# volume-em/empanada

Measured on AMD Instinct MI355X. Metric: Mvox/s end-to-end 3D panoptic inference (incl. consensus); PQ vs CPU ref, higher is better.
Workload: dtype f32

## Files before the change

empanada_amd/csrc/emp_conv.hip:

```cpp
#include "emp_common.h"
#include "emp_wino4.h"
#include <stdlib.h>

typedef float f32x16 __attribute__((ext_vector_type(16)));

#define CG_BM 128
#define CG_BK 32
#define CG_THREADS 256

struct ConvGeom {
    const float *x, *w, *scale, *shift, *res;
    float *out;
    int N, H, W, Cin, OH, OW, Cout, KH, KW, stride, pad, dil, relu;
    int64_t M, out_ps, res_ps;
    int tiles_m, tiles_n;
    int64_t x_bs, w_bs, out_bs;
    const int32_t *tiles;
    const float *proj_w;
    float *proj_out;
    int proj_n;
    int64_t hw;
};

__device__ __attribute__((aligned(16))) float cg_zero_page[64];
// ... 416 lines not shown
            }
            if constexpr (PROJ) {
                float ps[4] = {0.f, 0.f, 0.f, 0.f};
                if (valid && co + 3 < g.Cout) {
#pragma unroll
                    for (int q = 0; q < 4; ++q)
                        if (q < g.proj_n) {
                            const float4 wq = *reinterpret_cast<const float4 *>(g.proj_w + (int64_t)q * g.Cout + co);
                            ps[q] = __fadd_rn(__fadd_rn(__fadd_rn(__fmul_rn(v[0], wq.x), __fmul_rn(v[1], wq.y)),
                                                        __fmul_rn(v[2], wq.z)), __fmul_rn(v[3], wq.w));
                        }
                }
                *reinterpret_cast<float4 *>(&Cs[lrow_c * CLD + ccol]) = make_float4(ps[0], ps[1], ps[2], ps[3]);
            }
        }
        if constexpr (PROJ) {
            __syncthreads();
            for (int idx = tid; idx < EPI_ROWS * g.proj_n; idx += CG_THREADS) {
                const int row_l = idx / g.proj_n, q = idx - row_l * g.proj_n;
                const int64_t p = m0 + rd * EPI_ROWS + row_l;
                if (p < g.M) {
                    float t = Cs[row_l * CLD + q];
#pragma unroll 8
                    for (int j = 1; j < C4; ++j) t = __fadd_rn(t, Cs[row_l * CLD + 4 * j + q]);
                    const int64_t img = p / g.hw;
                    atomicAdd(g.proj_out + (img * g.proj_n + q) * g.hw + (p - img * g.hw), t);
                }
            }
        }
    }
}

struct CgPlan {
    bool narrow, respf, glds;
    int slab, tiles_m, tiles_n;
};

static CgPlan cg_plan(int64_t M, int Cout, int batch, bool has_res, bool res_vec_ok, bool may_split_n = true, int cin = 32)
{
    CgPlan p;
    const int64_t wide_blocks = emp_cdiv(M, CG_BM) * emp_cdiv(Cout, 128) * batch;
    p.narrow = Cout <= 64 || (Cout % 128 != 0 && Cout % 128 <= 64 && Cout < 512) || (may_split_n && wide_blocks < 256);
    p.tiles_m = (int)emp_cdiv(M, CG_BM);
    p.tiles_n = (int)emp_cdiv(Cout, p.narrow ? 64 : 128);
    static const char *fnarrow = getenv("EMP_CONV_NARROW");
    static const char *norespf = getenv("EMP_CONV_NO_RESPF");
    if (fnarrow && fnarrow[0] == '1') {
        p.narrow = true;
        p.tiles_n = (int)emp_cdiv(Cout, 64);
    }
    p.respf = has_res && res_vec_ok && Cout % (p.narrow ? 64 : 128) == 0 && !norespf;
    static const char *force = getenv("EMP_CONV_BK");
    const int64_t blocks = (int64_t)p.tiles_m * p.tiles_n * batch;
    p.slab = blocks > 512 ? 16 : 32;
    if (force && force[0] == '1') p.slab = 16;
    if (force && force[0] == '3') p.slab = 32;
    if (p.respf) p.slab = 32;
    if (cin % 32 != 0) {
        p.slab = 16;
        p.respf = false;
    }
    static const char *noglds = getenv("EMP_CONV_NO_GLDS");
    p.glds = !noglds;
    return p;
}

extern "C" int emp_conv_k_slab(int64_t M, int Cout, int batch, int has_residual)
{
    return cg_plan(M, Cout, batch, has_residual != 0, true).slab;
}

extern "C" int emp_conv_k_slab_cin(int64_t M, int Cout, int batch, int has_residual, int Cin)
{
    return cg_plan(M, Cout, batch, has_residual != 0, true, true, Cin).slab;
}

extern "C" __attribute__((visibility("hidden"))) int emp_conv1x1_ws_kind(int64_t M, int Cin, int Cout, int KH, int KW, int stride, int pad, int relu, int has_residual);
extern "C" __attribute__((visibility("hidden"))) int emp_conv1x1_ws_launch(int kind, const float *x, const float *w, const float *scale, const float *shift,
                                     const float *res, int64_t res_ps, int relu, int64_t M, int Cin, int Cout,
                                     float *out, int64_t out_ps, void *stream);
extern "C" __attribute__((visibility("hidden"))) int emp_gemm_ws_eligible(int batch, int64_t M, int N, int K, int slab);
extern "C" __attribute__((visibility("hidden"))) int emp_gemm_ws_launch(const float *A, const float *B, int batch, int64_t M, int N, int K, float *C,
                                                                        void *stream);

extern "C" int emp_conv_k_slab_geom(int64_t M, int Cout, int has_residual, int Cin, int KH, int KW, int stride, int pad,
                                    int relu)
{
    if (emp_conv1x1_ws_kind(M, Cin, Cout, KH, KW, stride, pad, relu, has_residual) == 1) return 64;
    return cg_plan(M, Cout, 1, has_residual != 0 && relu != 2, true, true, Cin).slab;
}

extern "C" int emp_conv_bn_act_nhwc(const float *x, const float *w_okkc, const float *scale, const float *shift,
                                    const float *residual, int64_t res_pixel_stride, int relu, int N, int H, int W,
                                    int Cin, int Cout, int KH, int KW, int stride, int pad, int dil, float *out,
                                    int64_t out_pixel_stride, void *stream)
{
    EMP_REQUIRE(x && w_okkc && out, "conv: null pointer");
    EMP_REQUIRE(N >= 0 && H > 0 && W > 0 && Cin > 0 && Cout > 0, "conv: bad shape");
    EMP_REQUIRE(Cin % 16 == 0, "conv: Cin %d must be a multiple of 16", Cin);
    EMP_REQUIRE(relu != 2 || residual, "conv: the gate epilogue (relu == 2) needs the gated tensor as residual");
    EMP_REQUIRE(KH >= 1 && KW >= 1 && KH <= 7 && KW <= 7 && stride >= 1 && dil >= 1 && pad >= 0, "conv: bad filter geometry");
    const int OH = (H + 2 * pad - dil * (KH - 1) - 1) / stride + 1;
    const int OW = (W + 2 * pad - dil * (KW - 1) - 1) / stride + 1;
    EMP_REQUIRE(OH > 0 && OW > 0, "conv: empty output");
    if (out_pixel_stride == 0) out_pixel_stride = Cout;
    if (res_pixel_stride == 0) res_pixel_stride = Cout;
    EMP_REQUIRE(out_pixel_stride >= Cout && res_pixel_stride >= Cout, "conv: bad pixel stride");
    EMP_REQUIRE(((reinterpret_cast<uintptr_t>(x) | reinterpret_cast<uintptr_t>(w_okkc)) & 15) == 0,
                "conv: x and w must be 16-byte aligned");
    EMP_REQUIRE(out != x, "conv: output cannot alias the input");
    if (N == 0) return EMP_OK;
    ConvGeom g;
    g.x = x; g.w = w_okkc; g.scale = scale; g.shift = shift; g.res = residual; g.out = out;
    g.N = N; g.H = H; g.W = W; g.Cin = Cin; g.OH = OH; g.OW = OW; g.Cout = Cout; g.KH = KH; g.KW = KW;
    g.stride = stride; g.pad = pad; g.dil = dil; g.relu = relu;
    g.M = (int64_t)N * OH * OW; g.out_ps = out_pixel_stride; g.res_ps = res_pixel_stride;
    g.x_bs = g.w_bs = g.out_bs = 0; g.tiles = nullptr; g.proj_w = nullptr; g.proj_out = nullptr; g.proj_n = 0; g.hw = 1;
    const bool res_vec_ok = (res_pixel_stride & 3) == 0 && (reinterpret_cast<uintptr_t>(residual) & 15) == 0;
    const bool io_vec_ok = res_vec_ok && (out_pixel_stride & 3) == 0 && (reinterpret_cast<uintptr_t>(out) & 15) == 0 &&
                           (!scale || (reinterpret_cast<uintptr_t>(scale) & 15) == 0) &&
                           (!shift || (reinterpret_cast<uintptr_t>(shift) & 15) == 0);
    const int ws = io_vec_ok && scale && shift ? emp_conv1x1_ws_kind(g.M, Cin, Cout, KH, KW, stride, pad, relu, residual != nullptr) : 0;
    if (ws == 1)
        return emp_conv1x1_ws_launch(1, x, w_okkc, scale, shift, residual, res_pixel_stride, relu, g.M, Cin, Cout, out,
                                     out_pixel_stride, stream);
    const CgPlan pl = cg_plan(g.M, Cout, 1, residual != nullptr && relu != 2, res_vec_ok, true, Cin);
    if (ws == 2 && !residual && pl.slab == 16)
        return emp_conv1x1_ws_launch(2, x, w_okkc, scale, shift, nullptr, res_pixel_stride, relu, g.M, Cin, Cout, out,
                                     out_pixel_stride, stream);
    if (ws == 3 && residual && pl.respf && pl.slab == 32 &&
        res_pixel_stride < (1 << 24) && out_pixel_stride < (1 << 24))
        return emp_conv1x1_ws_launch(3, x, w_okkc, scale, shift, residual, res_pixel_stride, relu, g.M, Cin, Cout, out,
                                     out_pixel_stride, stream);
    const bool narrow = pl.narrow, respf = pl.respf, bk16 = pl.slab == 16;
    EMP_REQUIRE((int64_t)pl.tiles_m * pl.tiles_n < (1LL << 28), "conv: too many tiles");
    g.tiles_m = pl.tiles_m;
    g.tiles_n = pl.tiles_n;
    const int T = g.tiles_m * g.tiles_n;
    const int grid = 8 * ((T + 7) / 8);
#define CG_GO(NT_, RES_, BK_, GL_) hipLaunchKernelGGL((conv_igemm_f32_kernel<NT_, 0, RES_, BK_, false, GL_>), dim3(grid), dim3(CG_THREADS), 0, emp_stream(stream), g)
#define CG_GATE(NT_, BK_) hipLaunchKernelGGL((conv_igemm_f32_kernel<NT_, 0, false, BK_, false, true, true>), dim3(grid), dim3(CG_THREADS), 0, emp_stream(stream), g)
    if (relu == 2) {
        if (narrow) { if (bk16) CG_GATE(1, 16); else CG_GATE(1, 32); }
        else { if (bk16) CG_GATE(2, 16); else CG_GATE(2, 32); }
    } else if (narrow) {
        if (respf) { if (pl.glds) CG_GO(1, true, 32, true); else CG_GO(1, true, 32, false); }
        else if (pl.glds) { if (bk16) CG_GO(1, false, 16, true); else CG_GO(1, false, 32, true); }
        else { if (bk16) CG_GO(1, false, 16, false); else CG_GO(1, false, 32, false); }
    } else {
        if (respf) { if (pl.glds) CG_GO(2, true, 32, true); else CG_GO(2, true, 32, false); }
        else if (pl.glds) { if (bk16) CG_GO(2, false, 16, true); else CG_GO(2, false, 32, true); }
        else { if (bk16) CG_GO(2, false, 16, false); else CG_GO(2, false, 32, false); }
    }
#undef CG_GO
#undef CG_GATE
    EMP_CHECK_LAUNCH("emp_conv_bn_act_nhwc");
    return EMP_OK;
}

__global__ __launch_bounds__(256) void splitk_reduce_kernel(const float *__restrict__ work, int nz, int64_t M, int Cout,
                                                            const float *__restrict__ scale,
                                                            const float *__restrict__ shift,
                                                            const float *__restrict__ res, int64_t res_ps, int relu,
                                                            float *__restrict__ out, int64_t out_ps)
{
    const int C4 = Cout >> 2;
// ... 33 lines not shown
    const int S = KH * KW * (Cin / 32);
    if (tiles > 128) return 1;
    int64_t k = 256 / tiles;
    if (k > S / 4) k = S / 4;
    if (k > 32) k = 32;
    return k >= 2 ? (int)k : 1;
}

extern "C" int emp_conv_splitk_bn_act_nhwc(const float *x, const float *w_okkc, const float *scale, const float *shift,
                                           const float *residual, int64_t res_pixel_stride, int relu, int N, int H, int W,
                                           int Cin, int Cout, int KH, int KW, int stride, int pad, int dil, int k_splits,
                                           float *work, float *out, int64_t out_pixel_stride, void *stream)
{
    EMP_REQUIRE(x && w_okkc && out && work, "conv_splitk: null pointer");
    EMP_REQUIRE(N >= 0 && H > 0 && W > 0 && Cin > 0 && Cout > 0, "conv_splitk: bad shape");
    EMP_REQUIRE(Cin % 32 == 0 && Cout % 4 == 0, "conv_splitk: Cin %d must be a multiple of 32, Cout %d of 4", Cin, Cout);
    EMP_REQUIRE(relu == 0 || relu == 1, "conv_splitk: relu must be 0 or 1");
    EMP_REQUIRE(KH >= 1 && KW >= 1 && KH <= 7 && KW <= 7 && stride >= 1 && dil >= 1 && pad >= 0, "conv_splitk: bad filter geometry");
    const int OH = (H + 2 * pad - dil * (KH - 1) - 1) / stride + 1;
    const int OW = (W + 2 * pad - dil * (KW - 1) - 1) / stride + 1;
    EMP_REQUIRE(OH > 0 && OW > 0, "conv_splitk: empty output");
    const int S = KH * KW * (Cin / 32);
    EMP_REQUIRE(k_splits >= 1 && k_splits <= S && k_splits <= 64, "conv_splitk: k_splits %d not in 1..min(%d, 64)", k_splits, S);
    if (out_pixel_stride == 0) out_pixel_stride = Cout;
    if (res_pixel_stride == 0) res_pixel_stride = Cout;
    EMP_REQUIRE(out_pixel_stride >= Cout && res_pixel_stride >= Cout, "conv_splitk: bad pixel stride");
    EMP_REQUIRE(((reinterpret_cast<uintptr_t>(x) | reinterpret_cast<uintptr_t>(w_okkc) | reinterpret_cast<uintptr_t>(work) |
                  reinterpret_cast<uintptr_t>(out) | reinterpret_cast<uintptr_t>(residual) | reinterpret_cast<uintptr_t>(scale) |
                  reinterpret_cast<uintptr_t>(shift)) & 15) == 0 && (out_pixel_stride & 3) == 0 && (res_pixel_stride & 3) == 0,
                "conv_splitk: pointers must be 16-byte aligned, pixel strides multiples of 4");
    EMP_REQUIRE(out != x && work != x && work != out, "conv_splitk: buffers must not alias");
    if (N == 0) return EMP_OK;
    ConvGeom g;
    g.x = x; g.w = w_okkc; g.scale = nullptr; g.shift = nullptr; g.res = nullptr; g.out = work;
    g.N = N; g.H = H; g.W = W; g.Cin = Cin; g.OH = OH; g.OW = OW; g.Cout = Cout; g.KH = KH; g.KW = KW;
    g.stride = stride; g.pad = pad; g.dil = dil; g.relu = 0;
    g.M = (int64_t)N * OH * OW; g.out_ps = Cout; g.res_ps = Cout;
    g.x_bs = g.w_bs = g.out_bs = 0; g.tiles = nullptr; g.proj_w = nullptr; g.proj_out = nullptr; g.proj_n = 0; g.hw = 1;
    const CgPlan pl = cg_plan(g.M, Cout, 1, false, true, true, Cin);
    EMP_REQUIRE((int64_t)pl.tiles_m * pl.tiles_n < (1LL << 28), "conv_splitk: too many tiles");
    g.tiles_m = pl.tiles_m;
    g.tiles_n = pl.tiles_n;
    const int T = g.tiles_m * g.tiles_n;
    const dim3 grid(8 * ((T + 7) / 8), 1, k_splits);
    hipStream_t st = emp_stream(stream);
    if (pl.narrow)
        hipLaunchKernelGGL((conv_igemm_f32_kernel<1, 0, false, 32, false, true>), grid, dim3(CG_THREADS), 0, st, g);
    else
        hipLaunchKernelGGL((conv_igemm_f32_kernel<2, 0, false, 32, false, true>), grid, dim3(CG_THREADS), 0, st, g);
    EMP_CHECK_LAUNCH("emp_conv_splitk_bn_act_nhwc(partials)");
    const int64_t total = g.M * (Cout / 4);
    hipLaunchKernelGGL(splitk_reduce_kernel, dim3(emp_grid(total, 256, 4096)), dim3(256), 0, st, work, k_splits, g.M, Cout,
                       scale, shift, residual, res_pixel_stride, relu, out, out_pixel_stride);
    EMP_CHECK_LAUNCH("emp_conv_splitk_bn_act_nhwc(reduce)");
    return EMP_OK;
}

extern "C" int emp_conv_bn_act_proj_nhwc(const float *x, const float *w_okkc, const float *scale, const float *shift,
                                         int relu, int N, int H, int W, int Cin, int Cout, int KH, int KW, int stride,
                                         int pad, int dil, const float *proj_w, int proj_n, float *proj_out,
                                         float *out, int64_t out_pixel_stride, void *stream)
{
    EMP_REQUIRE(x && w_okkc && proj_w && proj_out, "conv_proj: null pointer");
    EMP_REQUIRE(N >= 0 && H > 0 && W > 0 && Cin > 0 && Cin % CG_BK == 0, "conv_proj: bad shape (Cin %% %d)", CG_BK);
    EMP_REQUIRE(Cout == 128 || Cout == 256, "conv_proj: Cout %d must be 128 or 256 (at most two cout tiles)", Cout);
    EMP_REQUIRE(proj_n >= 1 && proj_n <= 4, "conv_proj: proj_n %d not in 1..4", proj_n);
    EMP_REQUIRE(KH >= 1 && KW >= 1 && KH <= 7 && KW <= 7 && stride >= 1 && dil >= 1 && pad >= 0, "conv_proj: bad filter geometry");
    const int OH = (H + 2 * pad - dil * (KH - 1) - 1) / stride + 1;
    const int OW = (W + 2 * pad - dil * (KW - 1) - 1) / stride + 1;
    EMP_REQUIRE(OH > 0 && OW > 0, "conv_proj: empty output");
    if (out_pixel_stride == 0) out_pixel_stride = Cout;
    EMP_REQUIRE(((reinterpret_cast<uintptr_t>(x) | reinterpret_cast<uintptr_t>(w_okkc) | reinterpret_cast<uintptr_t>(proj_w) |
                  reinterpret_cast<uintptr_t>(out)) & 15) == 0 && (out_pixel_stride & 3) == 0, "conv_proj: alignment");
    EMP_REQUIRE(out != x, "conv_proj: output cannot alias the input");
    if (N == 0) return EMP_OK;
    ConvGeom g;
    g.x = x; g.w = w_okkc; g.scale = scale; g.shift = shift; g.res = nullptr; g.out = out;
    g.N = N; g.H = H; g.W = W; g.Cin = Cin; g.OH = OH; g.OW = OW; g.Cout = Cout; g.KH = KH; g.KW = KW;
    g.stride = stride; g.pad = pad; g.dil = dil; g.relu = relu;
    g.M = (int64_t)N * OH * OW; g.out_ps = out_pixel_stride; g.res_ps = Cout;
    g.x_bs = g.w_bs = g.out_bs = 0; g.tiles = nullptr;
    g.proj_w = proj_w; g.proj_out = proj_out; g.proj_n = proj_n; g.hw = (int64_t)OH * OW;
    const CgPlan pl = cg_plan(g.M, Cout, 1, false, true, false);
    g.tiles_m = pl.tiles_m;
    g.tiles_n = pl.tiles_n;
    const int T = g.tiles_m * g.tiles_n;
    const int grid = 8 * ((T + 7) / 8);
#define CG_GOP(BK_, GL_) hipLaunchKernelGGL((conv_igemm_f32_kernel<2, 0, false, BK_, true, GL_>), dim3(grid), dim3(CG_THREADS), 0, emp_stream(stream), g)
    if (pl.glds) { if (pl.slab == 16) CG_GOP(16, true); else CG_GOP(32, true); }
    else { if (pl.slab == 16) CG_GOP(16, false); else CG_GOP(32, false); }
#undef CG_GOP
    EMP_CHECK_LAUNCH("emp_conv_bn_act_proj_nhwc");
    return EMP_OK;
}


__global__ __launch_bounds__(256) void wino_input_kernel(const float *__restrict__ x, const int32_t *__restrict__ tiles,
                                                         int64_t T, int H, int W, int C4, int dil, float4 *__restrict__ V)
{
    const int64_t total = T * C4;
    for (int64_t i = (int64_t)blockIdx.x * blockDim.x + threadIdx.x; i < total; i += (int64_t)gridDim.x * blockDim.x) {
        const int c4 = (int)(i % C4);
        const int64_t t = i / C4;
        const int n = tiles[3 * t], by = tiles[3 * t + 1], bx = tiles[3 * t + 2];
        const float4 *src = reinterpret_cast<const float4 *>(x) + (int64_t)n * H * W * C4 + c4;
        float4 d[4][4];
#pragma unroll
        for (int a = 0; a < 4; ++a)
#pragma unroll
            for (int b = 0; b < 4; ++b) {
                const int yy = by + a * dil, xx = bx + b * dil;
                d[a][b] = make_float4(0.f, 0.f, 0.f, 0.f);
                if (yy >= 0 && yy < H && xx >= 0 && xx < W) d[a][b] = src[((int64_t)yy * W + xx) * C4];
            }
#define W_SUB(p, q) make_float4(__fsub_rn(p.x, q.x), __fsub_rn(p.y, q.y), __fsub_rn(p.z, q.z), __fsub_rn(p.w, q.w))
#define W_ADD(p, q) make_float4(__fadd_rn(p.x, q.x), __fadd_rn(p.y, q.y), __fadd_rn(p.z, q.z), __fadd_rn(p.w, q.w))
        float4 tt[4][4];
#pragma unroll
        for (int a = 0; a < 4; ++a) {
            tt[a][0] = W_SUB(d[a][0], d[a][2]);
            tt[a][1] = W_ADD(d[a][1], d[a][2]);
            tt[a][2] = W_SUB(d[a][2], d[a][1]);
            tt[a][3] = W_SUB(d[a][1], d[a][3]);
        }
        float4 *dst = V + t * C4 + c4;
        const int64_t ps = T * C4;
#pragma unroll
        for (int v = 0; v < 4; ++v) {
            dst[(0 * 4 + v) * ps] = W_SUB(tt[0][v], tt[2][v]);
            dst[(1 * 4 + v) * ps] = W_ADD(tt[1][v], tt[2][v]);
            dst[(2 * 4 + v) * ps] = W_SUB(tt[2][v], tt[1][v]);
            dst[(3 * 4 + v) * ps] = W_SUB(tt[1][v], tt[3][v]);
        }
    }
}

__global__ __launch_bounds__(256) void wino_output_kernel(const float4 *__restrict__ Mw, const int32_t *__restrict__ tiles,
                                                          int64_t T, int H, int W, int Co4, int dil,
                                                          const float4 *__restrict__ scale, const float4 *__restrict__ shift,
                                                          int relu, float *__restrict__ out, int64_t out_ps)
{
    const int64_t total = T * Co4;
    for (int64_t i = (int64_t)blockIdx.x * blockDim.x + threadIdx.x; i < total; i += (int64_t)gridDim.x * blockDim.x) {
        const int c4 = (int)(i % Co4);
        const int64_t t = i / Co4;
        const int n = tiles[3 * t], oy = tiles[3 * t + 1] + dil, ox = tiles[3 * t + 2] + dil;
        const float4 *src = Mw + t * Co4 + c4;
        const int64_t ps = T * Co4;
        float4 m[4][4];
#pragma unroll
        for (int a = 0; a < 4; ++a)
#pragma unroll
            for (int b = 0; b < 4; ++b) m[a][b] = src[(a * 4 + b) * ps];
        float4 s[2][4];
#pragma unroll
        for (int b = 0; b < 4; ++b) {
            s[0][b] = W_ADD(W_ADD(m[0][b], m[1][b]), m[2][b]);
            s[1][b] = W_SUB(W_SUB(m[1][b], m[2][b]), m[3][b]);
        }
        float4 sc = make_float4(1.f, 1.f, 1.f, 1.f), sh = make_float4(0.f, 0.f, 0.f, 0.f);
        if (scale) sc = scale[c4];
        if (shift) sh = shift[c4];
#pragma unroll
        for (int a = 0; a < 2; ++a) {
            float4 yv[2];
            yv[0] = W_ADD(W_ADD(s[a][0], s[a][1]), s[a][2]);
// ... 367 lines not shown
```

empanada_amd/csrc/emp_conv1x1.hip:

```cpp
#include "emp_common.h"
#include <stdlib.h>
#include <atomic>
#include <type_traits>

typedef float f32x16 __attribute__((ext_vector_type(16)));
template <int V> using IC = std::integral_constant<int, V>;

#define PW_THREADS 256
#define PW_ROWS 32
#define PW_MIN_ROWS 65536
#define PW_MIN_ROWS_PLAN 262144

struct PwGeom {
    const float *x, *w, *scale, *shift, *res;
    float *out;
    int64_t M, out_ps, res_ps;
    int Cin, Cout, relu, groups, pix_blocks;
    int batch;
    int64_t x_bs, w_bs, out_bs;
};

template <int KS, int S, int CT, int PT, bool GEMM, bool RES, bool RELU, int MODE = 0>
__global__ __launch_bounds__(PW_THREADS, 1) void conv1x1_ws_kernel(PwGeom g)
{
    static_assert(MODE == 0 || RES, "MODE 1 is a residual form");
    constexpr int CIN = 64 * KS;
    constexpr int LD = CIN + 4;
    constexpr int BN = 32 * CT;
    constexpr int NQ = CIN / 8;
    constexpr int QS = S / 8;
    constexpr int ROWS = PW_ROWS * PT;
    static_assert(!RES || (CT == 4 && PT == 1 && !GEMM), "residual: 128-cout groups of the convolution form only");
    static_assert(S == 16 || S == 32 || S == 64, "K-slab");
    __shared__ __attribute__((aligned(16))) float Bs[BN * LD];

    const int bid = blockIdx.x;
    const int xcd = bid & 7, slot = bid >> 3;
    const int per_xcd = g.pix_blocks >> 3;
    const int gi = slot % g.groups;
    const int pb = xcd * per_xcd + slot / g.groups;
    const int n0 = GEMM ? 0 : gi * BN;
    const int tid = threadIdx.x;
    const float *xb = g.x, *wb = g.w;
    float *ob = g.out;

    auto stage = [&]() {
        for (int idx = tid; idx < BN * (CIN / 4); idx += PW_THREADS) {
            const int rr = idx / (CIN / 4), k4 = idx - rr * (CIN / 4);
            const int cw = n0 + CT * (rr & 31) + (rr >> 5);
            *reinterpret_cast<float4 *>(&Bs[rr * LD + 4 * k4]) = *reinterpret_cast<const float4 *>(wb + (int64_t)cw * CIN + 4 * k4);
        }
        __syncthreads();
    };

    const int wave = MODE != 0 ? __builtin_amdgcn_readfirstlane(tid >> 6) : tid >> 6, lane = tid & 63;
    const int r = lane & 31, hh = lane >> 5;
    const int co = n0 + CT * r;
    float sc[CT], sh[CT];
    if constexpr (!GEMM) {
        if constexpr (CT == 4) {
            { const float4 t = *reinterpret_cast<const float4 *>(g.scale + co); sc[0] = t.x; sc[1] = t.y; sc[2] = t.z; sc[3] = t.w; }
            { const float4 t = *reinterpret_cast<const float4 *>(g.shift + co); sh[0] = t.x; sh[1] = t.y; sh[2] = t.z; sh[3] = t.w; }
        } else {
            { const float2 t = *reinterpret_cast<const float2 *>(g.scale + co); sc[0] = t.x; sc[1] = t.y; }
            { const float2 t = *reinterpret_cast<const float2 *>(g.shift + co); sh[0] = t.x; sh[1] = t.y; }
        }
    }

    const int64_t n_tiles = (g.M + ROWS - 1) / ROWS;
    const int64_t n_full = g.M / ROWS;
    const float *Bl = &Bs[r * LD + hh * (S / 2)];
    const int64_t ops = GEMM ? (int64_t)BN : g.out_ps;
    const unsigned a_lane = r * CIN + hh * (S / 2);
    const unsigned r_lane = (unsigned)(4 * hh * g.res_ps + co), o_lane = (unsigned)(4 * hh * ops + co);

    auto load_a = [&](int64_t t, float4 (&a)[PT][NQ], const float *base) {
#pragma unroll
        for (int p = 0; p < PT; ++p) {
            const int64_t pa = t * ROWS + PW_ROWS * p + r;
            const float *ap = base + pa * CIN + hh * (S / 2);
#pragma unroll
            for (int i = 0; i < NQ; ++i) a[p][i] = *reinterpret_cast<const float4 *>(ap + S * (i / QS) + 4 * (i % QS));
        }
    };
    auto load_rs = [&](int64_t t, float4 (&rs)[RES ? 16 : 1]) {
        if constexpr (MODE == 1) {
            const float *rp = g.res + t * ROWS * g.res_ps;
#pragma unroll
            for (int q = 0; q < 16; ++q)
                rs[q] = *reinterpret_cast<const float4 *>(rp + (int64_t)((q & 3) + 8 * (q >> 2)) * g.res_ps + r_lane);
        } else if constexpr (RES) {
            const float *rp = g.res + (t * ROWS + 4 * hh) * g.res_ps + co;
#pragma unroll
            for (int q = 0; q < 16; ++q)
                rs[q] = *reinterpret_cast<const float4 *>(rp + (int64_t)((q & 3) + 8 * (q >> 2)) * g.res_ps);
        }
    };
    auto mma = [&](f32x16 (&acc)[PT * CT], const auto &a, auto i_lo_c, auto i_hi_c, auto a_off_c) {
        constexpr int i_lo = decltype(i_lo_c)::value, i_hi = decltype(i_hi_c)::value;
        constexpr int a_off = decltype(a_off_c)::value;
        if constexpr (i_lo == 0) {
#pragma unroll
            for (int j = 0; j < PT * CT; ++j)
#pragma unroll
                for (int q = 0; q < 16; ++q) acc[j][q] = 0.f;
        }
        int opaque = 0;
        asm volatile("" : "+v"(opaque));
        const float *Bt = Bl + opaque;
#pragma unroll
        for (int i = i_lo; i < i_hi; ++i) {
            float4 b[CT];
#pragma unroll
            for (int j = 0; j < CT; ++j) b[j] = *reinterpret_cast<const float4 *>(Bt + j * 32 * LD + S * (i / QS) + 4 * (i % QS));
#pragma unroll
            for (int e = 0; e < 4; ++e)
#pragma unroll
                for (int p = 0; p < PT; ++p) {
                    const float av = e == 0 ? a[p][i - a_off].x : e == 1 ? a[p][i - a_off].y : e == 2 ? a[p][i - a_off].z : a[p][i - a_off].w;
#pragma unroll
                    for (int j = 0; j < CT; ++j) {
                        const float bv = e == 0 ? b[j].x : e == 1 ? b[j].y : e == 2 ? b[j].z : b[j].w;
                        acc[p * CT + j] = __builtin_amdgcn_mfma_f32_32x32x2f32(av, bv, acc[p * CT + j], 0, 0, 0);
                    }
                }
        }
    };
    auto mma_all = [&](f32x16 (&acc)[PT * CT], const float4 (&a)[PT][NQ]) { mma(acc, a, IC<0>{}, IC<NQ>{}, IC<0>{}); };
    auto put = [&](float *dst, const f32x16 (&acc)[PT * CT], int p, const float4 (&rs)[RES ? 16 : 1], int q) {
        float v[CT];
#pragma unroll
        for (int e = 0; e < CT; ++e) v[e] = acc[p * CT + e][q];
        if constexpr (!GEMM) {
#pragma unroll
            for (int e = 0; e < CT; ++e) v[e] = __fadd_rn(__fmul_rn(v[e], sc[e]), sh[e]);
        }
        if constexpr (RES) {
            v[0] = __fadd_rn(v[0], rs[q].x); v[1] = __fadd_rn(v[1], rs[q].y);
            v[2] = __fadd_rn(v[2], rs[q].z); v[3] = __fadd_rn(v[3], rs[q].w);
        }
        if constexpr (RELU) {
#pragma unroll
            for (int e = 0; e < CT; ++e) v[e] = fmaxf(v[e], 0.f);
        }
        if constexpr (CT == 4) *reinterpret_cast<float4 *>(dst) = make_float4(v[0], v[1], v[2], v[3]);
        else *reinterpret_cast<float2 *>(dst) = make_float2(v[0], v[1]);
    };
    auto epi_part = [&](const f32x16 (&acc)[PT * CT], const float4 (&rs)[RES ? 16 : 1], int64_t t, auto q0_c, auto q1_c) {
#pragma unroll
        for (int p = 0; p < PT; ++p) {
            float *op = MODE != 0 ? ob + (t * ROWS + PW_ROWS * p) * ops : ob + (t * ROWS + PW_ROWS * p + 4 * hh) * ops + co;
#pragma unroll
            for (int q = decltype(q0_c)::value; q < decltype(q1_c)::value; ++q)
                put(op + (int64_t)((q & 3) + 8 * (q >> 2)) * ops + (MODE != 0 ? o_lane : 0u), acc, p, rs, q);
        }
    };
    auto epi = [&](const f32x16 (&acc)[PT * CT], const float4 (&rs)[RES ? 16 : 1], int64_t t) { epi_part(acc, rs, t, IC<0>{}, IC<16>{}); };

    auto run = [&](const int64_t t_first, const int64_t stride_t, const int64_t t_end) {
        const int64_t f_end = n_full < t_end ? n_full : t_end;
        if (t_first < f_end) {
            const int64_t m = (f_end - t_first + stride_t - 1) / stride_t;
            auto tile = [&](int64_t i) { return t_first + (i < m ? i : m - 1) * stride_t; };
            if constexpr (MODE == 0) {
                float4 a0[PT][NQ], a1[PT][NQ], rs0[RES ? 16 : 1], rs1[RES ? 16 : 1];
                f32x16 acc0[PT * CT], acc1[PT * CT];
                load_a(tile(0), a0, xb);
                load_rs(tile(0), rs0);
                load_a(tile(1), a1, xb);
                mma_all(acc0, a0);
                int64_t i = 1;
                for (; i + 1 < m; i += 2) {
                    load_rs(tile(i), rs1);
                    load_a(tile(i + 1), a0, xb);
                    mma_all(acc1, a1);
                    epi(acc0, rs0, tile(i - 1));
                    load_rs(tile(i + 1), rs0);
                    load_a(tile(i + 2), a1, xb);
                    mma_all(acc0, a0);
                    epi(acc1, rs1, tile(i));
                }
                if (i < m) {
                    load_rs(tile(i), rs1);
                    mma_all(acc1, a1);
                    epi(acc0, rs0, tile(i - 1));
                    epi(acc1, rs1, tile(i));
                } else {
                    epi(acc0, rs0, tile(i - 1));
                }
            } else if constexpr (MODE == 1) {
                constexpr int NE = NQ / 8;
                float4 a[PT][4 * NE], rs[16];
                f32x16 acc0[PT * CT], acc1[PT * CT];
                auto load_k = [&](int64_t t, auto slab_c) {
                    constexpr int off = decltype(slab_c)::value * NE, slot = (decltype(slab_c)::value & 3) * NE;
#pragma unroll
                    for (int p = 0; p < PT; ++p) {
                        const float *ap = xb + (t * ROWS + PW_ROWS * p) * CIN + a_lane;
#pragma unroll
                        for (int k = 0; k < NE; ++k) a[p][slot + k] = *reinterpret_cast<const float4 *>(ap + S * ((off + k) / QS) + 4 * ((off + k) % QS));
                    }
                };
                auto phase = [&](f32x16 (&acc_n)[PT * CT], int64_t t_n, const f32x16 (&acc_o)[PT * CT], int64_t t_o, auto with_epi, int64_t t_x, auto with_next) {
                    if constexpr (decltype(with_epi)::value) load_rs(t_o, rs);
                    auto eighth = [&](auto e_c) {
                        constexpr int E = decltype(e_c)::value;
                        mma(acc_n, a, IC<NE * E>{}, IC<NE * E + NE>{}, IC<NE * (E & 4)>{});
                        if constexpr (decltype(with_epi)::value && E >= 4) epi_part(acc_o, rs, t_o, IC<4 * (E - 4)>{}, IC<4 * (E - 4) + 4>{});
                        __builtin_amdgcn_sched_barrier(0);
                        if constexpr (E < 4) load_k(t_n, IC<E + 4>{});
                        else if constexpr (decltype(with_next)::value) load_k(t_x, IC<E - 4>{});
                    };
                    eighth(IC<0>{}); eighth(IC<1>{}); eighth(IC<2>{}); eighth(IC<3>{});
                    eighth(IC<4>{}); eighth(IC<5>{}); eighth(IC<6>{}); eighth(IC<7>{});
                };
                load_k(tile(0), IC<0>{}); load_k(tile(0), IC<1>{}); load_k(tile(0), IC<2>{}); load_k(tile(0), IC<3>{});
                phase(acc0, tile(0), acc1, 0, IC<0>{}, tile(1), IC<1>{});
                int64_t i = 1;
                for (; i + 1 < m; i += 2) {
                    phase(acc1, tile(i), acc0, tile(i - 1), IC<1>{}, tile(i + 1), IC<1>{});
                    phase(acc0, tile(i + 1), acc1, tile(i), IC<1>{}, tile(i + 2), IC<1>{});
                }
                if (i < m) {
                    phase(acc1, tile(i), acc0, tile(i - 1), IC<1>{}, 0, IC<0>{});
                    load_rs(tile(i), rs);
                    epi(acc1, rs, tile(i));
                } else {
                    load_rs(tile(i - 1), rs);
                    epi(acc0, rs, tile(i - 1));
                }
            }
        }
        if (n_full < t_end && n_full >= t_first && (n_full - t_first) % stride_t == 0) {
            const int64_t p0 = n_full * ROWS;
            float4 a[PT][NQ], rs[RES ? 16 : 1];
            f32x16 acc[PT * CT];
#pragma unroll
            for (int p = 0; p < PT; ++p) {
                const int64_t pr = p0 + PW_ROWS * p + r;
                const float *ap = xb + (pr < g.M ? pr : g.M - 1) * CIN + hh * (S / 2);
#pragma unroll
                for (int i = 0; i < NQ; ++i) a[p][i] = *reinterpret_cast<const float4 *>(ap + S * (i / QS) + 4 * (i % QS));
            }
            if constexpr (RES) {
#pragma unroll
                for (int q = 0; q < 16; ++q) {
                    int64_t p = p0 + (q & 3) + 8 * (q >> 2) + 4 * hh;
                    p = p < g.M ? p : g.M - 1;
                    rs[q] = *reinterpret_cast<const float4 *>(g.res + p * g.res_ps + co);
                }
            }
            mma_all(acc, a);
#pragma unroll
            for (int p = 0; p < PT; ++p)
#pragma unroll
                for (int q = 0; q < 16; ++q) {
                    const int64_t px = p0 + PW_ROWS * p + (q & 3) + 8 * (q >> 2) + 4 * hh;
                    if (px < g.M) put(ob + px * ops + co, acc, p, rs, q);
                }
        }
    };

    if constexpr (GEMM) {
        const int64_t G = (int64_t)g.batch * n_tiles;
        int64_t lo = G * bid / gridDim.x;
        const int64_t hi = G * (bid + 1) / gridDim.x;
        while (lo < hi) {
            const int64_t b = lo / n_tiles, t0 = lo - b * n_tiles;
            const int64_t t1 = hi - lo < n_tiles - t0 ? t0 + (hi - lo) : n_tiles;
            xb = g.x + b * g.x_bs;
            wb = g.w + b * g.w_bs;
            ob = g.out + b * g.out_bs;
            stage();
            run(t0 + wave, PW_THREADS / 64, t1);
            __syncthreads();
            lo += t1 - t0;
        }
    } else {
        stage();
        run((int64_t)pb * (PW_THREADS / 64) + wave, (int64_t)g.pix_blocks * (PW_THREADS / 64), n_tiles);
    }
}

static bool pw_off()
{
    static const char *off = getenv("EMP_CONV_NO_WS");
    return off && off[0] == '1';
}

static bool pw_off3()
{
    static const char *off = getenv("EMP_CONV_NO_WS3");
    return pw_off() || (off && off[0] == '1');
}

extern "C" __attribute__((visibility("hidden"))) int emp_conv1x1_ws_kind(int64_t M, int Cin, int Cout, int KH, int KW, int stride, int pad, int relu,
                                                                         int has_residual)
{
    if (pw_off()) return 0;
    if (!(KH == 1 && KW == 1 && stride == 1 && pad == 0 && relu != 2)) return 0;
    if ((Cin == 64 || Cin == 128) && Cout % 128 == 0 && Cout / 128 <= 8 && M >= PW_MIN_ROWS) return 1;
    if (!has_residual && M >= PW_MIN_ROWS_PLAN && ((Cin == 256 && Cout == 64) || (Cin == 64 && Cout == 64) || (Cin == 256 && Cout == 128)))
        return 2;
    if (has_residual && Cin == 256 && Cout % 128 == 0 && Cout / 128 <= 8 && M >= PW_MIN_ROWS && M * (Cout / 128) >= 8 * PW_MIN_ROWS &&
        !pw_off3())
        return 3;
    return 0;
}

extern "C" int emp_conv1x1_ws_eligible(int64_t M, int Cin, int Cout, int KH, int KW, int stride, int pad, int relu)
{
    return emp_conv1x1_ws_kind(M, Cin, Cout, KH, KW, stride, pad, relu, 0) != 0;
}

extern "C" __attribute__((visibility("hidden"))) int emp_gemm_ws_eligible(int batch, int64_t M, int N, int K, int slab)
{
    if (pw_off()) return 0;
    return (K == 64 || K == 128) && (N == 64 || N == 128) && slab == 16 && M >= PW_ROWS && (int64_t)batch * M >= PW_MIN_ROWS_PLAN;
}

template <int KS, int S, int CT, int PT, bool GEMM, bool RES, int MODE = 0>
static void pw_go(const PwGeom &g, int blocks, hipStream_t st)
{
    if (g.relu) {
        if constexpr (!GEMM) hipLaunchKernelGGL((conv1x1_ws_kernel<KS, S, CT, PT, GEMM, RES, true, MODE>), dim3(blocks), dim3(PW_THREADS), 0, st, g);
    } else {
        hipLaunchKernelGGL((conv1x1_ws_kernel<KS, S, CT, PT, GEMM, RES, false, MODE>), dim3(blocks), dim3(PW_THREADS), 0, st, g);
    }
}

static int pw_grid(PwGeom &g, int groups)
{
    g.groups = groups;
    int pix = 256 / groups;
    pix = pix / 8 * 8;
    if (pix < 8) pix = 8;
    g.pix_blocks = pix;
    return pix * groups;
}

static std::atomic<int64_t> pw_launches[4];

extern "C" int64_t emp_conv1x1_ws_launches(int kind)
{
    return kind >= 1 && kind <= 3 ? pw_launches[kind].load() : -1;
}

extern "C" __attribute__((visibility("hidden"))) int emp_conv1x1_ws_launch(int kind, const float *x, const float *w, const float *scale, const float *shift,
                                     const float *res, int64_t res_ps, int relu, int64_t M, int Cin, int Cout,
                                     float *out, int64_t out_ps, void *stream)
{
    PwGeom g;
    g.x = x; g.w = w; g.scale = scale; g.shift = shift; g.res = res; g.out = out;
    g.M = M; g.out_ps = out_ps; g.res_ps = res_ps; g.Cin = Cin; g.Cout = Cout; g.relu = relu;
    g.batch = 1; g.x_bs = g.w_bs = g.out_bs = 0;
    const int blocks = pw_grid(g, kind == 2 ? 1 : Cout / 128);
    hipStream_t st = emp_stream(stream);
    if (kind == 3) {
        pw_go<4, 32, 4, 1, false, true, 1>(g, blocks, st);
    } else if (kind == 1) {
        if (Cin == 64) { if (res) pw_go<1, 64, 4, 1, false, true>(g, blocks, st); else pw_go<1, 64, 4, 1, false, false>(g, blocks, st); }
        else { if (res) pw_go<2, 64, 4, 1, false, true>(g, blocks, st); else pw_go<2, 64, 4, 1, false, false>(g, blocks, st); }
    } else {
        if (Cin == 64) pw_go<1, 16, 2, 2, false, false>(g, blocks, st);
        else if (Cout == 64) pw_go<4, 16, 2, 1, false, false>(g, blocks, st);
        else pw_go<4, 16, 4, 1, false, false>(g, blocks, st);
    }
    EMP_CHECK_LAUNCH("emp_conv_bn_act_nhwc(1x1 weight-stationary)");
    pw_launches[kind]++;
    return EMP_OK;
}

extern "C" __attribute__((visibility("hidden"))) int emp_gemm_ws_launch(const float *A, const float *B, int batch, int64_t M, int N, int K, float *C,
                                                                        void *stream)
{
    PwGeom g;
    g.x = A; g.w = B; g.scale = g.shift = g.res = nullptr; g.out = C;
    g.M = M; g.out_ps = N; g.res_ps = N; g.Cin = K; g.Cout = N; g.relu = 0;
    g.batch = batch; g.x_bs = M * K; g.w_bs = (int64_t)N * K; g.out_bs = M * N;
    g.groups = 1; g.pix_blocks = 256;
    hipStream_t st = emp_stream(stream);
    if (K == 64) { if (N == 64) pw_go<1, 16, 2, 2, true, false>(g, 256, st); else pw_go<1, 16, 4, 1, true, false>(g, 256, st); }
    else { if (N == 64) pw_go<2, 16, 2, 2, true, false>(g, 256, st); else pw_go<2, 16, 4, 1, true, false>(g, 256, st); }
    EMP_CHECK_LAUNCH("emp_gemm_nt_batched(weight-stationary)");
    return EMP_OK;
}

extern "C" int emp_conv1x1_ws_kind_for(int64_t M, int Cin, int Cout, int KH, int KW, int stride, int pad, int relu, int has_residual)
{
    return emp_conv1x1_ws_kind(M, Cin, Cout, KH, KW, stride, pad, relu, has_residual);
}
```

Before: 133.5.

## Route 1x1 conv+projection heads through weight-stationary kernel with fused projection epilogue

Adds a projection-epilogue variant of the weight-stationary 1x1 conv kernel for Cin=256, Cout 128/256 when no full output is needed. BN/ReLU output is dotted with small projection weights in LDS, reduced per row, and atomically added into the projection output. The projection math is interleaved with the next tile's MFMA work in eighths to overlap it. This replaces the generic implicit-GEMM proj path, at the cost of extra LDS, atomics and a nondeterministic summation order.

```diff
diff --git a/empanada_amd/csrc/emp_conv.hip b/empanada_amd/csrc/emp_conv.hip
--- a/empanada_amd/csrc/emp_conv.hip
+++ b/empanada_amd/csrc/emp_conv.hip
@@ -522,6 +522,10 @@
 extern "C" __attribute__((visibility("hidden"))) int emp_gemm_ws_eligible(int batch, int64_t M, int N, int K, int slab);
 extern "C" __attribute__((visibility("hidden"))) int emp_gemm_ws_launch(const float *A, const float *B, int batch, int64_t M, int N, int K, float *C,
                                                                         void *stream);
+extern "C" __attribute__((visibility("hidden"))) int emp_conv1x1_ws_proj_eligible(int64_t M, int Cin, int Cout, int slab, int proj_n);
+extern "C" __attribute__((visibility("hidden"))) int emp_conv1x1_ws_proj_launch(const float *x, const float *w, const float *scale, const float *shift,
+                                                                                int relu, int64_t M, int64_t hw, int Cout, const float *proj_w,
+                                                                                int proj_n, float *proj_out, void *stream);
 
 extern "C" int emp_conv_k_slab_geom(int64_t M, int Cout, int has_residual, int Cin, int KH, int KW, int stride, int pad,
                                     int relu)
@@ -721,6 +725,10 @@
     g.x_bs = g.w_bs = g.out_bs = 0; g.tiles = nullptr;
     g.proj_w = proj_w; g.proj_out = proj_out; g.proj_n = proj_n; g.hw = (int64_t)OH * OW;
     const CgPlan pl = cg_plan(g.M, Cout, 1, false, true, false);
+    if (!out && KH == 1 && KW == 1 && stride == 1 && pad == 0 && dil == 1 && scale && shift &&
+        ((reinterpret_cast<uintptr_t>(scale) | reinterpret_cast<uintptr_t>(shift)) & 15) == 0 &&
+        emp_conv1x1_ws_proj_eligible(g.M, Cin, Cout, pl.slab, proj_n))
+        return emp_conv1x1_ws_proj_launch(x, w_okkc, scale, shift, relu, g.M, g.hw, Cout, proj_w, proj_n, proj_out, stream);
     g.tiles_m = pl.tiles_m;
     g.tiles_n = pl.tiles_n;
     const int T = g.tiles_m * g.tiles_n;
diff --git a/empanada_amd/csrc/emp_conv1x1.hip b/empanada_amd/csrc/emp_conv1x1.hip
--- a/empanada_amd/csrc/emp_conv1x1.hip
+++ b/empanada_amd/csrc/emp_conv1x1.hip
@@ -18,12 +18,16 @@
     int Cin, Cout, relu, groups, pix_blocks;
     int batch;
     int64_t x_bs, w_bs, out_bs;
+    const float *proj_w;
+    float *proj_out;
+    int64_t hw;
 };
 
-template <int KS, int S, int CT, int PT, bool GEMM, bool RES, bool RELU, int MODE = 0>
+template <int KS, int S, int CT, int PT, bool GEMM, bool RES, bool RELU, int MODE = 0, int PN = 0>
 __global__ __launch_bounds__(PW_THREADS, 1) void conv1x1_ws_kernel(PwGeom g)
 {
     static_assert(MODE == 0 || RES, "MODE 1 is a residual form");
+    static_assert(PN == 0 || (CT == 4 && PT == 1 && !GEMM && !RES && MODE == 0 && PN <= 3), "projection: 128-cout groups of the plain form");
     constexpr int CIN = 64 * KS;
     constexpr int LD = CIN + 4;
     constexpr int BN = 32 * CT;
@@ -33,6 +37,9 @@
     static_assert(!RES || (CT == 4 && PT == 1 && !GEMM), "residual: 128-cout groups of the convolution form only");
     static_assert(S == 16 || S == 32 || S == 64, "K-slab");
     __shared__ __attribute__((aligned(16))) float Bs[BN * LD];
+    constexpr int PLD = PW_ROWS + 1;
+    __shared__ float Ps[PN > 0 ? (PW_THREADS / 64) * PW_ROWS * PLD : 1];
+    __shared__ __attribute__((aligned(16))) float Pq[PN > 0 ? PN * BN : 4];
 
     const int bid = blockIdx.x;
     const int xcd = bid & 7, slot = bid >> 3;
@@ -155,7 +162,83 @@
                 put(op + (int64_t)((q & 3) + 8 * (q >> 2)) * ops + (MODE != 0 ? o_lane : 0u), acc, p, rs, q);
         }
     };
-    auto epi = [&](const f32x16 (&acc)[PT * CT], const float4 (&rs)[RES ? 16 : 1], int64_t t) { epi_part(acc, rs, t, IC<0>{}, IC<16>{}); };
+    struct ProjSums { float tot[PN > 0 ? PN : 1]; float *po; };
+    auto proj_slice = [&](const f32x16 (&acc)[PT * CT], ProjSums &ps, int64_t t, auto k_c) {
+        constexpr int k = decltype(k_c)::value, n = k / 2;
+        float *Pw = &Ps[(tid >> 6) * (PW_ROWS * PLD)];
+        if constexpr (k == 2 * PN) {
+            const unsigned p = (unsigned)(t * ROWS + r);
+            const unsigned img = p / (unsigned)g.hw;
+            ps.po = g.proj_out + (int64_t)img * PN * g.hw + (p - img * (unsigned)g.hw);
+        } else if constexpr (k % 2 == 0) {
+            const float4 wq = *reinterpret_cast<const float4 *>(&Pq[n * BN + CT * r]);
+            float scn[4];
+#pragma unroll
+            for (int e = 0; e < 4; ++e) scn[e] = sc[e];
+#pragma unroll
+            for (int e = 0; e < 4; ++e) asm volatile("" : "+v"(scn[e]));
+#pragma unroll
+            for (int q = 0; q < 16; ++q) {
+                float v[4];
+#pragma unroll
+                for (int e = 0; e < 4; ++e) {
+                    v[e] = __fadd_rn(__fmul_rn(acc[e][q], scn[e]), sh[e]);
+                    if constexpr (RELU) v[e] = fmaxf(v[e], 0.f);
+                }
+                Pw[((q & 3) + 8 * (q >> 2) + 4 * hh) * PLD + r] =
+                    __fadd_rn(__fadd_rn(__fadd_rn(__fmul_rn(v[0], wq.x), __fmul_rn(v[1], wq.y)), __fmul_rn(v[2], wq.z)), __fmul_rn(v[3], wq.w));
+            }
+            __builtin_amdgcn_fence(__ATOMIC_RELEASE, "wavefront");
+            __builtin_amdgcn_wave_barrier();
+        } else {
+            __builtin_amdgcn_fence(__ATOMIC_ACQUIRE, "wavefront");
+            float s = Pw[r * PLD];
+#pragma unroll
+            for (int j = 1; j < PW_ROWS; ++j) s = __fadd_rn(s, Pw[r * PLD + j]);
+            asm volatile("" : "+v"(s));
+            ps.tot[n] = s;
+            __builtin_amdgcn_fence(__ATOMIC_RELEASE, "wavefront");
+            __builtin_amdgcn_wave_barrier();
+            __builtin_amdgcn_fence(__ATOMIC_ACQUIRE, "wavefront");
+        }
+    };
+    auto commit = [&](const ProjSums &ps, int64_t t, bool partial) {
+        if (hh == 0 && (!partial || t * ROWS + r < g.M)) {
+#pragma unroll
+            for (int n = 0; n < PN; ++n) atomicAdd(ps.po + n * g.hw, ps.tot[n]);
+        }
+    };
+    auto epi_proj = [&](const f32x16 (&acc)[PT * CT], int64_t t, bool partial) {
+        if constexpr (PN > 0) {
+            ProjSums ps;
+            proj_slice(acc, ps, t, IC<0>{}); proj_slice(acc, ps, t, IC<1>{}); proj_slice(acc, ps, t, IC<2>{});
+            if constexpr (PN >= 2) { proj_slice(acc, ps, t, IC<3>{}); proj_slice(acc, ps, t, IC<4>{}); }
+            if constexpr (PN >= 3) { proj_slice(acc, ps, t, IC<5>{}); proj_slice(acc, ps, t, IC<6>{}); }
+            commit(ps, t, partial);
+        }
+    };
+    auto epi = [&](const f32x16 (&acc)[PT * CT], const float4 (&rs)[RES ? 16 : 1], int64_t t) {
+        if constexpr (PN > 0) epi_proj(acc, t, false);
+        else epi_part(acc, rs, t, IC<0>{}, IC<16>{});
+    };
+    auto mma_epi = [&](f32x16 (&acc_n)[PT * CT], const float4 (&a_n)[PT][NQ], const f32x16 (&acc_o)[PT * CT], const float4 (&rs_o)[RES ? 16 : 1], int64_t t_o) {
+        if constexpr (PN == 0) {
+            mma_all(acc_n, a_n);
+            epi(acc_o, rs_o, t_o);
+        } else {
+            static_assert(NQ % 8 == 0 && 2 * PN + 1 <= 8, "eighths");
+            ProjSums ps;
+            auto eighth = [&](auto e_c) {
+                constexpr int E = decltype(e_c)::value;
+                mma(acc_n, a_n, IC<NQ / 8 * E>{}, IC<NQ / 8 * E + NQ / 8>{}, IC<0>{});
+                if constexpr (E <= 2 * PN) proj_slice(acc_o, ps, t_o, e_c);
+                __builtin_amdgcn_sched_barrier(0);
+            };
+            eighth(IC<0>{}); eighth(IC<1>{}); eighth(IC<2>{}); eighth(IC<3>{});
+            eighth(IC<4>{}); eighth(IC<5>{}); eighth(IC<6>{}); eighth(IC<7>{});
+            commit(ps, t_o, false);
+        }
+    };
 
     auto run = [&](const int64_t t_first, const int64_t stride_t, const int64_t t_end) {
         const int64_t f_end = n_full < t_end ? n_full : t_end;
@@ -173,17 +256,14 @@
                 for (; i + 1 < m; i += 2) {
                     load_rs(tile(i), rs1);
                     load_a(tile(i + 1), a0, xb);
-                    mma_all(acc1, a1);
-                    epi(acc0, rs0, tile(i - 1));
+                    mma_epi(acc1, a1, acc0, rs0, tile(i - 1));
                     load_rs(tile(i + 1), rs0);
                     load_a(tile(i + 2), a1, xb);
-                    mma_all(acc0, a0);
-                    epi(acc1, rs1, tile(i));
+                    mma_epi(acc0, a0, acc1, rs1, tile(i));
                 }
                 if (i < m) {
                     load_rs(tile(i), rs1);
-                    mma_all(acc1, a1);
-                    epi(acc0, rs0, tile(i - 1));
+                    mma_epi(acc1, a1, acc0, rs0, tile(i - 1));
                     epi(acc1, rs1, tile(i));
                 } else {
                     epi(acc0, rs0, tile(i - 1));
@@ -237,8 +317,10 @@
             f32x16 acc[PT * CT];
 #pragma unroll
             for (int p = 0; p < PT; ++p) {
-                const int64_t pr = p0 + PW_ROWS * p + r;
-                const float *ap = xb + (pr < g.M ? pr : g.M - 1) * CIN + hh * (S / 2);
+                int ro = r, ho = hh;
+                if constexpr (PN > 0) asm volatile("" : "+v"(ro), "+v"(ho));
+                const int64_t pr = p0 + PW_ROWS * p + ro;
+                const float *ap = xb + (pr < g.M ? pr : g.M - 1) * CIN + ho * (S / 2);
 #pragma unroll
                 for (int i = 0; i < NQ; ++i) a[p][i] = *reinterpret_cast<const float4 *>(ap + S * (i / QS) + 4 * (i % QS));
             }
@@ -251,13 +333,17 @@
                 }
             }
             mma_all(acc, a);
-#pragma unroll
-            for (int p = 0; p < PT; ++p)
-#pragma unroll
-                for (int q = 0; q < 16; ++q) {
-                    const int64_t px = p0 + PW_ROWS * p + (q & 3) + 8 * (q >> 2) + 4 * hh;
-                    if (px < g.M) put(ob + px * ops + co, acc, p, rs, q);
-                }
+            if constexpr (PN > 0) {
+                epi_proj(acc, n_full, true);
+            } else {
+#pragma unroll
+                for (int p = 0; p < PT; ++p)
+#pragma unroll
+                    for (int q = 0; q < 16; ++q) {
+                        const int64_t px = p0 + PW_ROWS * p + (q & 3) + 8 * (q >> 2) + 4 * hh;
+                        if (px < g.M) put(ob + px * ops + co, acc, p, rs, q);
+                    }
+            }
         }
     };
 
@@ -277,6 +363,10 @@
             lo += t1 - t0;
         }
     } else {
+        if constexpr (PN > 0) {
+            if (tid < PN * (BN / 4))
+                *reinterpret_cast<float4 *>(&Pq[4 * tid]) = *reinterpret_cast<const float4 *>(g.proj_w + (int64_t)(tid / (BN / 4)) * g.Cout + n0 + 4 * (tid % (BN / 4)));
+        }
         stage();
         run((int64_t)pb * (PW_THREADS / 64) + wave, (int64_t)g.pix_blocks * (PW_THREADS / 64), n_tiles);
     }
@@ -291,6 +381,12 @@
 static bool pw_off3()
 {
     static const char *off = getenv("EMP_CONV_NO_WS3");
+    return pw_off() || (off && off[0] == '1');
+}
+
+static bool pw_off_k256()
+{
+    static const char *off = getenv("EMP_CONV_NO_WS_K256");
     return pw_off() || (off && off[0] == '1');
 }
 
@@ -319,13 +415,19 @@
     return (K == 64 || K == 128) && (N == 64 || N == 128) && slab == 16 && M >= PW_ROWS && (int64_t)batch * M >= PW_MIN_ROWS_PLAN;
 }
 
-template <int KS, int S, int CT, int PT, bool GEMM, bool RES, int MODE = 0>
+extern "C" __attribute__((visibility("hidden"))) int emp_conv1x1_ws_proj_eligible(int64_t M, int Cin, int Cout, int slab, int proj_n)
+{
+    return !pw_off_k256() && Cin == 256 && (Cout == 128 || Cout == 256) && slab == 16 && proj_n <= 3 && M < (1LL << 31) &&
+           M * (Cout / 128) >= 8 * PW_MIN_ROWS;
+}
+
+template <int KS, int S, int CT, int PT, bool GEMM, bool RES, int MODE = 0, int PN = 0>
 static void pw_go(const PwGeom &g, int blocks, hipStream_t st)
 {
     if (g.relu) {
-        if constexpr (!GEMM) hipLaunchKernelGGL((conv1x1_ws_kernel<KS, S, CT, PT, GEMM, RES, true, MODE>), dim3(blocks), dim3(PW_THREADS), 0, st, g);
+        if constexpr (!GEMM) hipLaunchKernelGGL((conv1x1_ws_kernel<KS, S, CT, PT, GEMM, RES, true, MODE, PN>), dim3(blocks), dim3(PW_THREADS), 0, st, g);
     } else {
-        hipLaunchKernelGGL((conv1x1_ws_kernel<KS, S, CT, PT, GEMM, RES, false, MODE>), dim3(blocks), dim3(PW_THREADS), 0, st, g);
+        hipLaunchKernelGGL((conv1x1_ws_kernel<KS, S, CT, PT, GEMM, RES, false, MODE, PN>), dim3(blocks), dim3(PW_THREADS), 0, st, g);
     }
 }
 
@@ -339,11 +441,11 @@
     return pix * groups;
 }
 
-static std::atomic<int64_t> pw_launches[4];
+static std::atomic<int64_t> pw_launches[5];
 
 extern "C" int64_t emp_conv1x1_ws_launches(int kind)
 {
-    return kind >= 1 && kind <= 3 ? pw_launches[kind].load() : -1;
+    return kind >= 1 && kind <= 4 ? pw_launches[kind].load() : -1;
 }
 
 extern "C" __attribute__((visibility("hidden"))) int emp_conv1x1_ws_launch(int kind, const float *x, const float *w, const float *scale, const float *shift,
@@ -354,6 +456,7 @@
     g.x = x; g.w = w; g.scale = scale; g.shift = shift; g.res = res; g.out = out;
     g.M = M; g.out_ps = out_ps; g.res_ps = res_ps; g.Cin = Cin; g.Cout = Cout; g.relu = relu;
     g.batch = 1; g.x_bs = g.w_bs = g.out_bs = 0;
+    g.proj_w = nullptr; g.proj_out = nullptr; g.hw = 1;
     const int blocks = pw_grid(g, kind == 2 ? 1 : Cout / 128);
     hipStream_t st = emp_stream(stream);
     if (kind == 3) {
@@ -371,6 +474,29 @@
     return EMP_OK;
 }
 
+extern "C" __attribute__((visibility("hidden"))) int emp_conv1x1_ws_proj_launch(const float *x, const float *w, const float *scale, const float *shift,
+                                                                                int relu, int64_t M, int64_t hw, int Cout, const float *proj_w,
+                                                                                int proj_n, float *proj_out, void *stream)
+{
+    EMP_REQUIRE(M > 0 && M < (1LL << 31) && hw > 0 && hw <= M, "conv_proj(1x1 weight-stationary): M %lld, hw %lld", (long long)M, (long long)hw);
+    PwGeom g;
+    g.x = x; g.w = w; g.scale = scale; g.shift = shift; g.res = nullptr; g.out = nullptr;
+    g.M = M; g.out_ps = Cout; g.res_ps = Cout; g.Cin = 256; g.Cout = Cout; g.relu = relu;
+    g.batch = 1; g.x_bs = g.w_bs = g.out_bs = 0;
+    g.proj_w = proj_w; g.proj_out = proj_out; g.hw = hw;
+    const int blocks = pw_grid(g, Cout / 128);
+    hipStream_t st = emp_stream(stream);
+    switch (proj_n) {
+    case 1: pw_go<4, 16, 4, 1, false, false, 0, 1>(g, blocks, st); break;
+    case 2: pw_go<4, 16, 4, 1, false, false, 0, 2>(g, blocks, st); break;
+    case 3: pw_go<4, 16, 4, 1, false, false, 0, 3>(g, blocks, st); break;
+    default: EMP_REQUIRE(false, "conv_proj(1x1 weight-stationary): proj_n %d not in 1..3", proj_n);
+    }
+    EMP_CHECK_LAUNCH("emp_conv_bn_act_proj_nhwc(1x1 weight-stationary)");
+    pw_launches[4]++;
+    return EMP_OK;
+}
+
 extern "C" __attribute__((visibility("hidden"))) int emp_gemm_ws_launch(const float *A, const float *B, int batch, int64_t M, int N, int K, float *C,
                                                                         void *stream)
 {
@@ -378,6 +504,7 @@
     g.x = A; g.w = B; g.scale = g.shift = g.res = nullptr; g.out = C;
     g.M = M; g.out_ps = N; g.res_ps = N; g.Cin = K; g.Cout = N; g.relu = 0;
     g.batch = batch; g.x_bs = M * K; g.w_bs = (int64_t)N * K; g.out_bs = M * N;
+    g.proj_w = nullptr; g.proj_out = nullptr; g.hw = 1;
     g.groups = 1; g.pix_blocks = 256;
     hipStream_t st = emp_stream(stream);
     if (K == 64) { if (N == 64) pw_go<1, 16, 2, 2, true, false>(g, 256, st); else pw_go<1, 16, 4, 1, true, false>(g, 256, st); }
```

Result: no change. 134.8, median of 6 (+0.9%).
